# spaceml-org/STARCOP

Hardware: AMD Instinct MI355X
Metric: 512x512 hyperspectral tiles/sec (train fwd+bwd) (higher is better)
Workload: dtype f32; 1 GPU; configs[1]: HyperSTARCOP U-Net (smp.Unet mobilenet_v2, 4ch mag1c+RGB) train step fwd+loss+bwd+Adam, 512x512 tiles, fp32 HIP kernels (3x3 convs: fp32 operands split exactly into 16-bit terms on the matrix cores, fp32 accumulation; see config.precision and DESIGN.md section 2); batch_per_gpu=16, global_batch=16, parallelism=dp1, hipgraph=False, precision=fp32

## Files before the change

### include/starcop_hip.h

```cpp
#ifndef STARCOP_HIP_H
#define STARCOP_HIP_H

#include <stddef.h>
#include <stdint.h>

#ifdef __cplusplus
extern "C" {
#endif

typedef void* sc_stream;

enum sc_status {
  SC_OK = 0,
  SC_ERR_ARG = -1,
  SC_ERR_LAUNCH = -2,
  SC_ERR_NOTPD = -3,
  SC_ERR_NODEV = -4
};

enum sc_src_mode {
  SC_SRC_RAW = 0,
  SC_SRC_AFFINE = 1,
  SC_SRC_BNBWD = 2,
  SC_SRC_NORM = 3
// ... 86 lines not shown
  const float* part; float* dw;
  int32_t nparts, taps, Cout, Cin, CoP, CiP;
  uint64_t total;
} sc_wgrad_pending;
int sc_conv2d_wgrad_mfma_deferred(const sc_wgrad_args* a, sc_wgrad_pending* pending_host, sc_stream stream);
int sc_wgrad_reduce_batch(const sc_wgrad_pending* descs_dev, const uint32_t* block_starts_dev, int n, uint32_t total_blocks,
                          sc_stream stream);
#define SC_PACK_THIN16 5
#define SC_PACK_PW3 6
size_t sc_packed_weight_floats_thin16(int Cout, int Cin, int transpose_flip);
int sc_pack_weights_thin16(const float* w_oihw, float* wpk, int Cout, int Cin, int transpose_flip, sc_stream stream);
int sc_conv3x3_thin16(const sc_conv_args* a, sc_stream stream);

#define SC_PACK_SP 7
size_t sc_packed_weight_floats_sp(int Cout, int Cup, int Cskip);
int sc_pack_weights_sp(const float* w_oihw, float* wpk, int Cout, int Cup, int Cskip, int terms, sc_stream stream);
int sc_sp_stat_rows(int N, int H, int W, int Cout);
int sc_conv3x3_sp(const sc_conv_args* a, sc_stream stream);
#define SC_PACK_SPD 8
size_t sc_packed_weight_floats_spd(int Cout, int Cup, int Cskip_tiles );
int sc_spd_vskip_ok(int Cup, int Cskip);
int sc_pack_weights_spd(const float* w_oihw, float* wpk, int Cout, int CinTotal, int Cup, int vskip, int terms, sc_stream stream);
int sc_conv3x3_sp_dgrad(const sc_conv_args* a, sc_stream stream);
size_t sc_sp_wgrad_workspace_bytes(int N, int H, int W, int Cout, int Cup);
int sc_conv3x3_sp_wgrad(const sc_wgrad_args* a, void* ws, size_t ws_bytes, sc_stream stream);
int sc_wgrad_scatter_cols(const float* src, float* dw, int Cout, int Ccols, int CinTotal, int col_off, sc_stream stream);

size_t sc_wgrad_thin16_workspace_floats(int N, int H, int W, int Cout, int Cin);
int sc_conv3x3_wgrad_thin16(const sc_wgrad_args* a, sc_stream stream);

size_t sc_packed_weight_floats_pw3(int Cout, int Cin, int transpose_flip);
int sc_conv1x1_pw3(const sc_conv_args* a, sc_stream stream);
int sc_conv1x1_pw3_variant(int N, int H, int W, int Cout);
size_t sc_wgrad_pw3_workspace_floats(int N, int H, int W, int Cout, int Cin);
int sc_conv1x1_wgrad_pw3(const sc_wgrad_args* a, sc_wgrad_pending* pending_host, sc_stream stream);
int sc_wgrad_pw3_variant(int N, int H, int W, int Cout, int Cin);

typedef struct sc_irb_args {
  sc_src x;
  const float* wpk_expand;
  const float* cst_expand;
  const float* w_dw;
  const float* cst_dw;
  const float* wpk_project;
  const float* cst_project;
  float* out;
  float* z_absmax;
  int32_t N, Cin, hidden, Cout, H, W, stride, residual;
} sc_irb_args;
int sc_irb_supported(int Cin, int hidden, int Cout, int H, int W, int stride);
int sc_irb_variant(int Cin, int hidden, int Cout, int stride);
int sc_irb_eval(const sc_irb_args* a, sc_stream stream);

typedef struct sc_irt_args {
  sc_src x;
  const float* w_expand;
  const float* w_dw;
  const float* cst_expand;
  int32_t N, Cin, hidden, H, W, stride;
} sc_irt_args;
int sc_irt_supported(int Cin, int hidden, int H, int W, int stride);
int sc_irt_rows(int stage, int N, int H, int W, int stride);
int sc_irt_bwd_rows(int N, int hidden, int H, int W);
size_t sc_irt_bwd_workspace_floats(int N, int Cin, int hidden, int H, int W);
int sc_irt_expand_stats(const sc_irt_args* a, float* stats , sc_stream stream);
int sc_irt_fwd(const sc_irt_args* a, float* d_out , float* stats_d , sc_stream stream);
// ... 532 lines not shown
```

### starcop_amd/_lib.py

```python
import ctypes as C
import os
import subprocess

import torch

_HERE = os.path.dirname(os.path.abspath(__file__))
LIB_PATH = os.path.join(_HERE, "libstarcop_hip.so")
CSRC = os.path.join(_HERE, "csrc")

SC_CST = 8
STAT_CONV3, STAT_CONV1, STAT_DW, STAT_STEM, STAT_BNBWD, STAT_CONV1K, STAT_PW3 = 0, 1, 2, 3, 4, 5, 6

SRC_RAW, SRC_AFFINE, SRC_BNBWD, SRC_NORM = 0, 1, 2, 3
ACT_NONE, ACT_RELU, ACT_RELU6 = 0, 1, 2


class StarcopHipError(RuntimeError):
    pass


class sc_src(C.Structure):
    _fields_ = [("x", C.c_void_p), ("aux", C.c_void_p), ("cst", C.c_void_p),
                ("C", C.c_int32), ("mode", C.c_int32), ("act", C.c_int32), ("up", C.c_int32)]

# ... 317 lines not shown
    "sc_scene_gather_planes": (_i, [C.POINTER(sc_scene_planes_args), _vp]),
    "sc_scene_core_counts": (_i, [_vp, C.c_int64, C.c_int64, _i, _i, C.c_uint32, _vp, _vp, _i, _vp, _vp]),
    "sc_head_conv_fwd_mosaic_prob": (_i, [C.POINTER(sc_src), _vp, _vp, _vp, C.c_int64, _vp, C.c_int64, _i, _i, _vp, C.c_int64, C.c_int64,
                                          C.c_uint32, _f, _vp, _vp, _i, _i, _i, _i, _vp]),
    "sc_connected_components": (_i, [_vp, _i, _vp, _vp, _vp, _sz, _i, _i, _i, _vp]),
    "sc_proposed_mask": (_i, [_vp, C.c_int64, _vp, C.c_int64, _f, _i, _vp, _vp, _sz, _i, _i, _i, _vp]),
    "sc_packed_weight_floats_thin16": (_sz, [_i, _i, _i]),
    "sc_pack_weights_thin16": (_i, [_vp, _vp, _i, _i, _i, _vp]),
    "sc_conv3x3_thin16": (_i, [C.POINTER(sc_conv_args), _vp]),
    "sc_packed_weight_floats_sp": (_sz, [_i, _i, _i]),
    "sc_pack_weights_sp": (_i, [_vp, _vp, _i, _i, _i, _i, _vp]),
    "sc_sp_stat_rows": (_i, [_i, _i, _i, _i]),
    "sc_conv3x3_sp": (_i, [C.POINTER(sc_conv_args), _vp]),
    "sc_packed_weight_floats_spd": (_sz, [_i, _i, _i]),
    "sc_pack_weights_spd": (_i, [_vp, _vp, _i, _i, _i, _i, _i, _vp]),
    "sc_spd_vskip_ok": (_i, [_i, _i]),
    "sc_conv3x3_sp_dgrad": (_i, [C.POINTER(sc_conv_args), _vp]),
    "sc_sp_wgrad_workspace_bytes": (_sz, [_i, _i, _i, _i, _i]),
    "sc_conv3x3_sp_wgrad": (_i, [C.POINTER(sc_wgrad_args), _vp, _sz, _vp]),
    "sc_wgrad_scatter_cols": (_i, [_vp, _vp, _i, _i, _i, _i, _vp]),
    "sc_binary_opening": (_i, [_vp, _f, _i, _vp, _vp, _i, _i, _i, _vp]),
    "sc_threshold_confusion": (_i, [_vp, _vp, _vp, _vp, _i, _i, _vp, _vp, _i, _i, _i, _vp]),
    "sc_gather_augment": (_i, [_vp, _i, _i, _i, _i, _vp, _vp, _vp, _vp, _vp, _vp, _i, _i, _i, _i, _vp, _vp]),
    "sc_tile_window_sums": (_i, [_vp, _i, _i, _i, _vp, _vp, _i, _vp, _vp]),
    "sc_dwconv3x3_bwd_fused": (_i, [C.POINTER(sc_src), C.POINTER(sc_src), _vp, _vp, _vp, _vp, _i, _i, _i, _i, _i, _vp]),
    "sc_dw_variant": (_i, [_i, _i, _i, _i, _i, _i, _i]),
    "sc_wgrad_thin16_workspace_floats": (_sz, [_i, _i, _i, _i, _i]),
    "sc_conv3x3_wgrad_thin16": (_i, [C.POINTER(sc_wgrad_args), _vp]),
    "sc_conv2d_wgrad_mfma_deferred": (_i, [C.POINTER(sc_wgrad_args), C.POINTER(sc_wgrad_pending), _vp]),
    "sc_wgrad_reduce_batch": (_i, [_vp, _vp, _i, C.c_uint32, _vp]),
    "sc_packed_weight_floats_pw3": (_sz, [_i, _i, _i]),
    "sc_conv1x1_pw3": (_i, [C.POINTER(sc_conv_args), _vp]),
    "sc_conv1x1_pw3_variant": (_i, [_i, _i, _i, _i]),
    "sc_wgrad_pw3_workspace_floats": (_sz, [_i, _i, _i, _i, _i]),
    "sc_wgrad_pw3_variant": (_i, [_i, _i, _i, _i, _i]),
    "sc_conv1x1_wgrad_pw3": (_i, [C.POINTER(sc_wgrad_args), C.POINTER(sc_wgrad_pending), _vp]),
    "sc_irb_supported": (_i, [_i, _i, _i, _i, _i, _i]),
    "sc_irb_variant": (_i, [_i, _i, _i, _i]),
    "sc_irb_eval": (_i, [C.POINTER(sc_irb_args), _vp]),
    "sc_irt_supported": (_i, [_i, _i, _i, _i, _i]),
    "sc_irt_rows": (_i, [_i, _i, _i, _i, _i]),
    "sc_irt_bwd_rows": (_i, [_i, _i, _i, _i]),
    "sc_irt_bwd_workspace_floats": (_sz, [_i, _i, _i, _i, _i]),
    "sc_irt_expand_stats": (_i, [C.POINTER(sc_irt_args), _vp, _vp]),
    "sc_irt_fwd": (_i, [C.POINTER(sc_irt_args), _vp, _vp, _vp]),
    "sc_irt_bwd": (_i, [C.POINTER(sc_irt_args), C.POINTER(sc_src), _vp, _vp, _vp, _vp]),
    "sc_irt_xmoments": (_i, [C.POINTER(sc_irt_args), _vp, _vp]),
    "sc_irt_bwd_fix": (_i, [C.POINTER(sc_irt_args), _vp, _vp, _vp, _vp, _i, _vp]),
    "sc_irt_wgrad_finalize": (_i, [C.POINTER(sc_irt_args), _vp, _vp, _vp, _vp]),
    "sc_maxpool2x2": (_i, [C.POINTER(sc_src), _vp, _i, _i, _i, _i, _vp]),
    "sc_upsample_bilinear2x": (_i, [C.POINTER(sc_src), _vp, _i, _i, _i, _i, _vp]),
    "sc_maxpool2x2_bwd": (_i, [C.POINTER(sc_src), _vp, _vp, _i, _i, _i, _i, _i, _vp]),
    "sc_upsample_bilinear2x_bwd": (_i, [_vp, _vp, _i, _i, _i, _i, _vp]),
    "sc_pwreg_param_floats": (_sz, [_i, _i, _i, _i]),
    "sc_pwreg_fwd": (_i, [_vp, _vp, _i, _i, _i, _i, _i, _i, _i, _vp, _vp]),
    "sc_reg_loss": (_i, [_vp, _vp, _sz, _i, _vp, _vp, _vp, _vp]),
    "sc_pwreg_sweep_blocks": (_i, [_i, _i, _i]),
    "sc_pwreg_train_sweep": (_i, [_vp, _vp, _vp, _i, _i, _i, _i, _i, _i, _i, _i, _vp, _vp]),
    "sc_pwreg_finalize": (_i, [_vp, _i, _vp, _i, _i, _i, _i, _d, _vp, _vp, _vp]),
    "sc_panel_minmax": (_i, [_vp, C.POINTER(sc_panel), _i, _vp, _vp]),
    "sc_render_panels": (_i, [_vp, C.POINTER(sc_panel), _i, _vp, _vp, _i, _i, _vp]),
    "sc_component_stats_workspace_bytes": (_sz, [_i, _i, _i, _i, _i]),
    "sc_component_stats": (_i, [C.POINTER(sc_cstats_args), _vp, _sz, _vp]),
    "sc_component_outlines_workspace_bytes": (_sz, [_i, _i, C.c_int64]),
    "sc_component_outlines_rounds": (_i, [C.c_int64]),
    "sc_component_outlines": (_i, [C.POINTER(sc_outline_args), _i, _vp]),
# ... 106 lines not shown
```

### starcop_amd/csrc/conv_pw3.hip

```cpp
#include "sc_split.h"

namespace {

struct PwP {
  SrcD s;
  const uintx4* wpk;
  int NP, HW, K, M, nks, npb;
  float* out; const float* add0; int accum; float* stats;
  const float* bnr_y; const float* bnr_cst; float* bnr_rows; int bnr_act;
};

template <int NCB, int PD, bool BNB>
__global__ __launch_bounds__(256) void k_pw3(const PwP p) {
  constexpr int CW = BNB ? 8 : 2;
  extern __shared__ __attribute__((aligned(16))) float s_cst[];
  const int tid = threadIdx.x, lane = tid & 63, wave = tid >> 6;
  const int l31 = lane & 31, lhi = lane >> 5;
  const int HW = p.HW, K = p.K, M = p.M, nks = p.nks;
  for (int c = tid; c < nks * 16; c += 256) {
    if (BNB) {
      float4 c0 = make_float4(0.f, 0.f, 0.f, 0.f); float c4 = 0.f;
      if (c < K) { c0 = *reinterpret_cast<const float4*>(p.s.cst + (size_t)c * SC_CST); c4 = p.s.cst[(size_t)c * SC_CST + 4]; }
      *reinterpret_cast<float4*>(s_cst + c * 8) = c0;
      *reinterpret_cast<float4*>(s_cst + c * 8 + 4) = make_float4(c4, 0.f, 0.f, 0.f);
// ... 43 lines not shown

  for (int ks0 = 0; ks0 < nks; ks0 += PD) {
#pragma unroll
    for (int s = 0; s < PD; ++s) {
      const int ks = ks0 + s;
      const int kc = ks < nks ? ks : nks - 1;
      const bool live = pok && ks < nks;
      float v[8];
      if (BNB) {
        const float4* q = reinterpret_cast<const float4*>(s_cst + (kc * 16 + lhi * 8) * 8);
#pragma unroll
        for (int j = 0; j < 8; ++j) {
          const float4 c0 = q[2 * j]; const float c4 = q[2 * j + 1].x;
          const float t = sc_pro_bnbwd(xr[s][j], yr[BNB ? s : 0][j], c0.x, c0.y, c0.z, c0.w, c4, lo, hi);
          v[j] = live ? t : 0.f;
        }
      } else {
        const float4* q = reinterpret_cast<const float4*>(s_cst + (kc * 16 + lhi * 8) * 2);
#pragma unroll
        for (int jj = 0; jj < 4; ++jj) {
          const float4 c = q[jj];
          const float t0 = sc_pro_affine(xr[s][2 * jj], c.x, c.y, lo, hi), t1 = sc_pro_affine(xr[s][2 * jj + 1], c.z, c.w, lo, hi);
          v[2 * jj] = live ? t0 : 0.f;
          v[2 * jj + 1] = live ? t1 : 0.f;
        }
      }
      uintx4 a[3];
      split8(v, a);
#pragma unroll
      for (int m = 0; m < NCB; ++m) acc[m] = mfma6(a, br[s][m], acc[m]);
      PW3_ISSUE(s, ks + PD)
    }
  }
#undef PW3_ISSUE

  const bool vec4 = (HW & 3) == 0;
  unsigned ooff[4]; bool ook[4];
#pragma unroll
  for (int j = 0; j < 4; ++j) {
    const int g = pb * 32 + 8 * j + 4 * lhi;
    ook[j] = g < p.NP;
    const int gc = ook[j] ? g : 0;
    const int n_ = gc / HW;
    ooff[j] = (unsigned)(n_ * M) * (unsigned)HW + (unsigned)(gc - n_ * HW);
  }
#pragma unroll
  for (int m = 0; m < NCB; ++m) {
    const int co = (cbase + m) * 32 + l31;
    const bool cok = co < M;
    if (p.stats) {
      float s1 = 0.f, s2 = 0.f;
#pragma unroll
      for (int r = 0; r < 16; ++r) { s1 += acc[m][r]; s2 = fmaf(acc[m][r], acc[m][r], s2); }
      s1 += __shfl_xor(s1, 32, 64);
      s2 += __shfl_xor(s2, 32, 64);
      if (lhi == 0 && cok) *reinterpret_cast<float2*>(p.stats + ((size_t)pb * M + co) * 2) = make_float2(s1, s2);
    }
    if (!cok) continue;
    if (BNB && p.bnr_y != nullptr) {
      const float4 cb = *reinterpret_cast<const float4*>(p.bnr_cst + (size_t)co * SC_CST);
      const float blo = sc_act_lo(p.bnr_act), bhi = sc_act_hi(p.bnr_act);
      float yv[16];
#pragma unroll
      for (int r = 0; r < 16; ++r) yv[r] = 0.f;
      if (vec4) {
#pragma unroll
        for (int j = 0; j < 4; ++j) {
// ... 16 lines not shown
        const float gq = (g < p.NP && yh > blo && yh < bhi) ? acc[m][r] : 0.f;
        s1 += gq;
        s2 = fmaf(gq, (yv[r] - cb.z) * cb.w, s2);
      }
      s1 += __shfl_xor(s1, 32, 64);
      s2 += __shfl_xor(s2, 32, 64);
      if (lhi == 0) *reinterpret_cast<float2*>(p.bnr_rows + ((size_t)pb * M + co) * 2) = make_float2(s1, s2);
    }
    if (vec4) {
#pragma unroll
      for (int j = 0; j < 4; ++j) {
        if (!ook[j]) continue;
        const unsigned idx = ooff[j] + (unsigned)co * (unsigned)HW;
        float4 o = make_float4(acc[m][4 * j], acc[m][4 * j + 1], acc[m][4 * j + 2], acc[m][4 * j + 3]);
        if (p.add0) { const float4 t = *reinterpret_cast<const float4*>(p.add0 + idx); o.x += t.x; o.y += t.y; o.z += t.z; o.w += t.w; }
        if (p.accum) { const float4 t = *reinterpret_cast<const float4*>(p.out + idx); o.x += t.x; o.y += t.y; o.z += t.z; o.w += t.w; }
        *reinterpret_cast<float4*>(p.out + idx) = o;
      }
    } else {
#pragma unroll
      for (int r = 0; r < 16; ++r) {
        const int g = pb * 32 + 8 * (r >> 2) + 4 * lhi + (r & 3);
        if (g >= p.NP) continue;
        const int n_ = g / HW;
        const size_t idx = ((size_t)n_ * M + co) * HW + (g - n_ * HW);
        float o = acc[m][r];
        if (p.add0) o += p.add0[idx];
        if (p.accum) o += p.out[idx];
        p.out[idx] = o;
      }
    }
  }
}

struct PwWP {
  SrcD dy, s;
  int NP, HW, Cout, Cin;
  int ksteps;
  int per_wg;
  int CoP, CiP;
  float* part;
};

template <int TM, int TN, int PD>
__global__ __launch_bounds__(256) void k_pw3_wgrad(const PwWP p) {
  extern __shared__ __attribute__((aligned(16))) float s_red[];
  const int tid = threadIdx.x, lane = tid & 63, wave = tid >> 6;
  const int l31 = lane & 31, lhi = lane >> 5;
  const int HW = p.HW;
  const int mb0 = blockIdx.y * TM, nb0 = blockIdx.z * TN;
  float d_sc[TM], d_sh[TM], d_A[TM], d_B[TM], d_D[TM]; bool d_ok[TM]; unsigned d_c[TM];
  float x_sc[TN], x_sh[TN]; bool x_ok[TN]; unsigned x_c[TN];
  const bool dy_bnb = p.dy.mode == SC_SRC_BNBWD;
#pragma unroll
  for (int m = 0; m < TM; ++m) {
    const int co = (mb0 + m) * 32 + l31;
    d_ok[m] = co < p.Cout;
    d_c[m] = d_ok[m] ? co : 0;
    const float4 c0 = *reinterpret_cast<const float4*>(p.dy.cst + (size_t)d_c[m] * SC_CST);
    d_sc[m] = c0.x; d_sh[m] = c0.y; d_A[m] = c0.z; d_B[m] = c0.w; d_D[m] = p.dy.cst[(size_t)d_c[m] * SC_CST + 4];
  }
#pragma unroll
  for (int q = 0; q < TN; ++q) {
    const int ci = (nb0 + q) * 32 + l31;
    x_ok[q] = ci < p.Cin;
    x_c[q] = x_ok[q] ? ci : 0;
// ... 162 lines not shown
  SC_REQUIRE(((uintptr_t)a->wpk & 15) == 0, "sc_conv1x1_pw3: packed filters must be 16-byte aligned");
  const long NP = (long)a->N * a->H * a->W;
  SC_REQUIRE(NP * (long)(a->Cout > a->src[0].C ? a->Cout : a->src[0].C) < (1L << 32), "sc_conv1x1_pw3: tensor too large for 32-bit element offsets");
  PwP p;
  p.s = to_srcd(a->src[0]);
  if (p.s.mode == SC_SRC_RAW) {
    p.s.cst = sc_identity_cst_table(p.s.C);
    SC_REQUIRE(p.s.cst != nullptr, "sc_conv1x1_pw3: identity constants unavailable (C = %d)", p.s.C);
    p.s.act = SC_ACT_NONE;
  }
  p.wpk = reinterpret_cast<const uintx4*>(a->wpk);
  p.NP = (int)NP; p.HW = a->H * a->W; p.K = a->src[0].C; p.M = a->Cout;
  p.nks = (p.K + 15) / 16;
  p.npb = (int)((NP + 31) / 32);
  p.out = a->out0; p.add0 = a->add0; p.accum = a->accum0; p.stats = a->stats;
  p.bnr_y = nullptr; p.bnr_cst = nullptr; p.bnr_rows = nullptr; p.bnr_act = SC_ACT_NONE;
  if (a->bnr) {
    SC_REQUIRE(p.s.mode == SC_SRC_BNBWD && !a->add0 && !a->accum0 && !a->stats, "sc_conv1x1_pw3: sc_bnr_args go with a data-gradient launch that writes the complete gradient");
    SC_REQUIRE(a->bnr->y && a->bnr->cst && a->bnr->rows && !a->bnr->absmax, "sc_conv1x1_pw3: sc_bnr_args need y, cst and rows (no range hint on this path)");
    p.bnr_y = a->bnr->y; p.bnr_cst = a->bnr->cst; p.bnr_rows = a->bnr->rows; p.bnr_act = a->bnr->act;
  }
  const int MB = (p.M + 31) / 32;
  const int ncb = sc_conv1x1_pw3_variant(a->N, a->H, a->W, a->Cout);
  const bool bnb = p.s.mode == SC_SRC_BNBWD;
  dim3 grid((p.npb + 3) / 4, (MB + ncb - 1) / ncb);
  const size_t lds = (size_t)p.nks * 16 * (bnb ? 8 : 2) * sizeof(float);
  hipStream_t st = (hipStream_t)stream;
#define SC_PW(NCB, PD, B) hipLaunchKernelGGL((k_pw3<NCB, PD, B>), grid, dim3(256), lds, st, p)
  if (ncb == 4) { if (bnb) SC_PW(4, 2, true); else SC_PW(4, 2, false); }
  else if (ncb == 2) { if (bnb) SC_PW(2, 4, true); else SC_PW(2, 4, false); }
  else { if (bnb) SC_PW(1, 4, true); else SC_PW(1, 4, false); }
#undef SC_PW
  SC_LAUNCH_OK("sc_conv1x1_pw3");
  return SC_OK;
}

extern "C" size_t sc_wgrad_pw3_workspace_floats(int N, int H, int W, int Cout, int Cin) {
  const PwWPlan pl = plan_pw3_wgrad(N, H, W, Cout, Cin);
  const size_t E = (size_t)pl.CoP * pl.CiP;
  return (size_t)pl.nparts * E + sc_reduce_scratch_floats(pl.nparts, E);
}

extern "C" int sc_wgrad_pw3_variant(int N, int H, int W, int Cout, int Cin) {
  if (N <= 0 || H <= 0 || W <= 0 || Cout <= 0 || Cin <= 0) return -1;
  const PwWPlan pl = plan_pw3_wgrad(N, H, W, Cout, Cin);
  return 10 * pl.tm + pl.tn;
}

extern "C" int sc_conv1x1_wgrad_pw3(const sc_wgrad_args* a, sc_wgrad_pending* pending, sc_stream stream) {
  SC_REQUIRE(a != nullptr, "sc_conv1x1_wgrad_pw3: null args");
  SC_REQUIRE(a->ks == 1 && a->nsrc == 1, "sc_conv1x1_wgrad_pw3: ks must be 1 with a single source");
  SC_REQUIRE(a->src[0].C == a->Cin && a->dy.C == a->Cout, "sc_conv1x1_wgrad_pw3: channel mismatch");
  SC_REQUIRE(a->dy.up == 0 && a->src[0].up == 0, "sc_conv1x1_wgrad_pw3: sources cannot be upsampled");
  SC_REQUIRE(a->src[0].mode == SC_SRC_RAW || a->src[0].mode == SC_SRC_AFFINE, "sc_conv1x1_wgrad_pw3: input must be a RAW or AFFINE source");
  SC_REQUIRE(a->dy.mode != SC_SRC_NORM && (a->dy.mode != SC_SRC_BNBWD || a->dy.aux), "sc_conv1x1_wgrad_pw3: bad dy source");
  SC_REQUIRE((a->H * a->W) % 8 == 0, "sc_conv1x1_wgrad_pw3: H*W must be a multiple of 8 (got %d)", a->H * a->W);
  const PwWPlan pl = plan_pw3_wgrad(a->N, a->H, a->W, a->Cout, a->Cin);
  const size_t need = sc_wgrad_pw3_workspace_floats(a->N, a->H, a->W, a->Cout, a->Cin);
  SC_REQUIRE(a->part_floats >= need, "sc_conv1x1_wgrad_pw3: workspace too small (%zu < %zu floats)", a->part_floats, need);
  PwWP p;
  p.dy = to_srcd(a->dy); p.s = to_srcd(a->src[0]);
  if (p.dy.mode == SC_SRC_RAW) { p.dy.cst = sc_identity_cst_table(p.dy.C); p.dy.act = SC_ACT_NONE; SC_REQUIRE(p.dy.cst, "sc_conv1x1_wgrad_pw3: identity constants unavailable"); }
  if (p.s.mode == SC_SRC_RAW) { p.s.cst = sc_identity_cst_table(p.s.C); p.s.act = SC_ACT_NONE; SC_REQUIRE(p.s.cst, "sc_conv1x1_wgrad_pw3: identity constants unavailable"); }
  p.NP = a->N * a->H * a->W; p.HW = a->H * a->W; p.Cout = a->Cout; p.Cin = a->Cin;
  p.ksteps = pl.ksteps; p.per_wg = pl.per_wg; p.CoP = pl.CoP; p.CiP = pl.CiP; p.part = a->part;
  dim3 grid(pl.nparts, pl.CoP / (32 * pl.tm), pl.CiP / (32 * pl.tn));
// ... 18 lines not shown
```

### starcop_amd/network.py

```python
import collections
import ctypes as C
import math
import os

import torch
import torch.nn as nn

from . import _lib, scene
from ._lib import (ACT_NONE, ACT_RELU, ACT_RELU6, SC_CST, sc_irb_args, sc_irt_args, SRC_AFFINE, SRC_BNBWD, SRC_NORM, SRC_RAW, STAT_BNBWD, sc_wgrad_pending,
                   PACK_PW3, PACK_SP, PACK_SPD, PACK_THIN16, STAT_PW3, STAT_CONV1, STAT_CONV1K, STAT_CONV3, STAT_DW, STAT_STEM, TERMS_F16X2, check, make_src, ptr, sc_bn_tail, sc_bnr_args,
                   sc_conv_args, sc_wgrad_args, stream)

MBV2_SETTINGS = ((1, 16, 1, 1), (6, 24, 2, 2), (6, 32, 3, 2), (6, 64, 4, 2),
                 (6, 96, 3, 1), (6, 160, 3, 2), (6, 320, 1, 1))
DECODER_CHANNELS = (256, 128, 64, 32, 16)
BN_EPS, BN_MOMENTUM = 1e-5, 0.1
HeadMosaic = collections.namedtuple("HeadMosaic", "win win_host classes prob mask valid fill_bits nodata", defaults=(None,) * 4 + (0, 0.0))


def _conv_bn_act(cin, cout, k, stride=1, groups=1, act="relu6"):
    return nn.Sequential(nn.Conv2d(cin, cout, k, stride, (k - 1) // 2, groups=groups, bias=False),
                         nn.BatchNorm2d(cout, eps=BN_EPS, momentum=BN_MOMENTUM),
                         nn.ReLU6() if act == "relu6" else nn.ReLU())

# ... 145 lines not shown
    if _SP == "0" or Ho % 2 or Wo % 2:
        return False
    if _SP == "all":
        return True
    Hl, Wl = Ho // 2, Wo // 2
    tw = 32 if Wl >= 32 else 16
    wgs = N * (-(-Wl // tw)) * (-(-Hl // (256 // tw))) * (-(-Cout // 32))
    return Cout >= 32 and wgs >= 128


def _use_spd(N, Ho, Wo, Cup, Csk=0):
    if _SP == "0" or Ho % 2 or Wo % 2:
        return False
    return _SP == "all" or Cup >= 128 or (Csk and _lib.load().sc_spd_vskip_ok(Cup, Csk))


def _use_spd_skip_tiles(Cup, Csk):
    if _SP == "all":
        return True
    return _SP != "0" and _SP_SKIPTILES and Cup >= 1024 and -(-Csk // 32) * 3 <= -(-Cup // 128)


def _use_spw(N, Ho, Wo, Cout, Cup):
    if _SP == "0" or Ho % 2 or Wo % 2:
        return False
    return _SP == "all" or Cup >= 512


def _use_ksplit(N, HW, K, M, ks=1):
    if ks != 1:
        return False
    wgs = N * (-(-HW // 128)) * (-(-M // _pick_cot(M, 1)))
    return wgs <= 512 and (K >= 384 or (K >= 192 and wgs <= 256))


class HyperStarcopUNet(nn.Module):

    def __init__(self, in_channels=4, classes=1):
        super().__init__()
        if not (1 <= classes <= self.MAX_CLASSES):
            raise ValueError(f"HyperStarcopUNet: classes must be in [1, {self.MAX_CLASSES}] (sc_head_conv_fwd_k)")
        if not (1 <= in_channels <= self.MAX_IN_CHANNELS):
            raise ValueError(f"HyperStarcopUNet: in_channels must be in [1, {self.MAX_IN_CHANNELS}] (sc_stem_conv_fwd)")
        self.in_channels, self.classes = in_channels, classes
        self.encoder = _Encoder(in_channels)
        self.decoder = _Decoder()
        self.segmentation_head = nn.Sequential(nn.Conv2d(DECODER_CHANNELS[-1], classes, 3, padding=1))
        self.reset_parameters()
        self._ops, self._tensors = self._build_ops()
        self._plans = {}
        self._pflat = self._gflat = None
        self._pack_version = None
        self.register_load_state_dict_post_hook(HyperStarcopUNet._after_load)

    MAX_IN_CHANNELS, MAX_CLASSES = 16, 8
    MAX_TRAIN_IN_CHANNELS, MAX_TRAIN_CLASSES = 8, 1

    @staticmethod
    def _after_load(module, incompatible_keys):
        module.check_split_range()

    FP16_MAX_WEIGHT, FP16_MAX_ACT = 255.0, 32752.0
    range_check_every = 200

    def _split_feeders(self):
        raw, fin = [], []
# ... 211 lines not shown
    class _Plan:
        pass

    def _get_plan(self, N, H, W, need_grad, want_logits=True, want_classes=None):
        want_classes = (not want_logits) if want_classes is None else want_classes
        key = (N, H, W)
        plan = self._plans.get(key)
        dev = self._pflat.device
        if plan is None:
            plan = HyperStarcopUNet._Plan()
            plan.N, plan.H, plan.W = N, H, W
            plan.buf, plan.grad = {}, {}
            f32 = dict(dtype=torch.float32, device=dev)
            lib = _lib.load()
            plan.cst, plan.cstb, plan.stats_v, plan.bsums_v, plan.srows, plan.brows = {}, {}, {}, {}, {}, {}
            kind_of = {"stem": STAT_STEM, "dw": STAT_DW, "conv3": STAT_CONV3, "pw": STAT_CONV1}
            plan.irt, plan.irt_of_dw, plan.irt_rows = {}, {}, {}
            if self.fuse_irt:
                for i_e, (i_dw, i_pr, stride) in self._ir_blocks.items():
                    cv, tin = self._ops[i_e]["conv"], self._ops[i_e]["ins"][0]
                    if tin.kind != "input" and _use_irt(N, cv.in_channels, cv.out_channels, H >> tin.shift, W >> tin.shift, stride):
                        plan.irt[i_e], plan.irt_of_dw[i_dw] = i_dw, i_e
                        te, td = self._ops[i_e]["out"], self._ops[i_dw]["out"]
                        plan.irt_rows[te.name] = lib.sc_irt_rows(0, N, H >> tin.shift, W >> tin.shift, stride)
                        plan.irt_rows[td.name] = lib.sc_irt_rows(1, N, H >> tin.shift, W >> tin.shift, stride)
            irt_e = {self._ops[i]["out"].name for i in plan.irt}
            for op in self._ops:
                t = op["out"]
                if t.kind != "input" and t.name not in plan.buf and t.name not in irt_e and t.name != "logits":
                    plan.buf[t.name] = torch.empty((N, t.C, H >> t.shift, W >> t.shift), **f32)
                if t.bn is not None:
                    Ho, Wo = H >> t.shift, W >> t.shift
                    kind = kind_of[op["type"]]
                    if op["type"] == "pw" and _use_pw3(0, N, Ho * Wo, op["conv"].in_channels, op["conv"].out_channels):
                        kind = STAT_PW3
                    elif op["type"] == "pw" and _use_ksplit(N, Ho * Wo, op["conv"].in_channels, op["conv"].out_channels):
                        kind = STAT_CONV1K
                    plan.srows[t.name] = max(lib.sc_stat_rows(kind, N, Ho, Wo), plan.irt_rows.get(t.name, 0))
                    plan.brows[t.name] = lib.sc_stat_rows(STAT_BNBWD, N, Ho, Wo)
                    plan.stats_v[t.name] = torch.empty(plan.srows[t.name] * t.C * 2, **f32)
                    plan.cst[t.name] = torch.zeros((t.C, SC_CST), **f32)
                    plan.cstb[t.name] = torch.zeros((t.C, SC_CST), **f32)
            plan.irb = {}
            for i_e, (i_dw, i_pr, stride) in self._ir_blocks.items():
                cv_e, cv_p, tin = self._ops[i_e]["conv"], self._ops[i_pr]["conv"], self._ops[i_e]["ins"][0]
                if tin.kind != "input" and _use_irb(N, cv_e.in_channels, cv_e.out_channels, cv_p.out_channels, H >> tin.shift, W >> tin.shift, stride):
                    i_add = i_pr + 1 if (i_pr + 1 < len(self._ops) and self._ops[i_pr + 1]["type"] == "add"
                                         and self._ops[i_pr + 1]["ins"][1] is self._ops[i_pr]["out"]) else None
                    plan.irb[i_e] = (i_dw, i_pr, i_add)
                    lay = getattr(self, "_irb_layers", None)
                    if lay is None:
                        lay = self._irb_layers = set()
                    if not {i_e, i_pr} <= lay:
                        lay.update((i_e, i_pr))
                        self._pack_version = None
                        self._pack_tables = {}
            need = getattr(self, "_pw_need", None)
            if need is None:
                need = self._pw_need = {}
            for i, op in enumerate(self._ops):
                if op["type"] == "pw":
                    hw = (H >> op["out"].shift) * (W >> op["out"].shift)
                    for tflip in (0, 1):
                        cv = op["conv"]
                        lay = "pw3" if _use_pw3(tflip, N, hw, cv.in_channels, cv.out_channels) else "mfma"
                        if lay not in need.setdefault((i, tflip), set()):
                            need[(i, tflip)].add(lay)
                            self._pack_version = None
                            self._pack_tables = {}
            fins = [t.name for t in self._tensors.values() if t.kind == "fin" and t.name != "logits"]
            plan.bn_scratch = torch.empty(64 * 2 * max(t.C for t in self._tensors.values()), dtype=torch.float64, device=dev)
            plan.fin_slot = {n: i for i, n in enumerate(fins)}
            plan.fin_amax = torch.zeros(len(fins), **f32)
            raw_feed = self._split_feeders()[0]
            plan.act_slot = {n: i for i, n in enumerate(raw_feed)}
            plan.act_amax = torch.zeros(max(len(raw_feed), 1), **f32)
            plan.n_eval = 0
            plan.has_grad = False
            self._plans[key] = plan
        if want_logits and "logits" not in plan.buf:
            plan.buf["logits"] = torch.empty((N, self.classes, H, W), dtype=torch.float32, device=dev)
        if want_classes and getattr(plan, "classes", None) is None:
            plan.classes = torch.empty((N, H, W), dtype=torch.uint8, device=dev)
        if need_grad and not plan.has_grad:
            lib = _lib.load()
            f32 = dict(dtype=torch.float32, device=dev)
            ws, up = 0, 0
            n_dw = 0
            irt_e = {self._ops[i]["out"].name for i in plan.irt}
            plan.irt_esums, plan.irt_work = {}, {}
            for i_e in plan.irt:
                cv, tin, te = self._ops[i_e]["conv"], self._ops[i_e]["ins"][0], self._ops[i_e]["out"]
                Hi, Wi = H >> tin.shift, W >> tin.shift
                plan.irt_esums[te.name] = torch.empty(lib.sc_irt_bwd_rows(N, cv.out_channels, Hi, Wi) * cv.out_channels * 2, dtype=torch.float64, device=dev)
                plan.irt_work[te.name] = torch.empty(lib.sc_irt_bwd_workspace_floats(N, cv.in_channels, cv.out_channels, Hi, Wi), **f32)
            for op in self._ops:
                o = op["out"]
                Ho, Wo = H >> o.shift, W >> o.shift
# ... 344 lines not shown
                    xb_ = self._xbound(plan, o)
                    bt.act_bound = xb_.value if xb_ is not None else None
                    check(lib.sc_dwconv3x3_fwd_bn(C.byref(s), ptr(conv.weight), ptr(plan.buf[o.name]), N, o.C,
                                                  H >> tin.shift, W >> tin.shift, op["stride"], stats, C.byref(bt), st))
                    bn_done = True
                else:
                    check(lib.sc_dwconv3x3_fwd(C.byref(s), ptr(conv.weight), ptr(plan.buf[o.name]), N, o.C,
                                               H >> tin.shift, W >> tin.shift, op["stride"], stats, st))
            elif ty in ("pw", "conv3"):
                if ty == "conv3" and self._late_pack_stream is not None:
                    check(lib.sc_stream_wait_stream(st, self._late_pack_stream))
                    self._late_pack_stream = None
                a = sc_conv_args()
                ins = op["ins"]
                a.nsrc = len(ins)
                a.src[0] = self._src_of(plan, ins[0], up=1 if op.get("up") else 0)
                if len(ins) == 2:
                    a.src[1] = self._src_of(plan, ins[1])
                ent = self._wpk[i]
                a.wpk = ent["f"].data_ptr()
                a.N, a.H, a.W, a.Cout = N, Ho, Wo, o.C
                a.ks, a.co_t = conv.kernel_size[0], ent["cot_f"]
                a.out0 = plan.buf[o.name].data_ptr(); a.out1 = None
                a.csplit, a.accum0, a.accum1 = o.C, 0, 0
                a.add0 = None; a.add1 = None
                a.stats = plan.stats_v[o.name].data_ptr() if stats is not None else None
                a.terms = ent["terms_f"]
                if ty == "conv3":
                    for k_, t_ in enumerate(ins):
                        a.xbound[k_] = self._xbound(plan, t_)
                if ty == "pw" and _use_pw3(0, N, Ho * Wo, conv.in_channels, conv.out_channels):
                    fconv = lib.sc_conv1x1_pw3
                    a.wpk = ent["pf"].data_ptr()
                elif (op.get("up") and ent.get("sp") is not None and ent["terms_f"] in _SP_TERMS and self.split_bf16
                      and _use_sp(N, Ho, Wo, o.C)):
                    fconv = lib.sc_conv3x3_sp
                    a.wpk = ent["sp"].data_ptr()
                    srows = lib.sc_sp_stat_rows(N, Ho, Wo, o.C)
                elif ent["tf"] is not None:
                    fconv = lib.sc_conv3x3_thin16
                    a.wpk = ent["tf"].data_ptr()
                elif ent["bx3_f"]:
                    fconv = lib.sc_conv3x3_bx3
                elif _use_ksplit(N, Ho * Wo, conv.in_channels, conv.out_channels, a.ks):
                    fconv = lib.sc_conv1x1_ksplit
                else:
                    fconv = lib.sc_conv2d_mfma
                check(fconv(C.byref(a), st))
            elif ty == "add":
                sa = self._src_of(plan, op["ins"][0])
                sb = self._src_of(plan, op["ins"][1])
                check(lib.sc_add_srcs_absmax(C.byref(sa), C.byref(sb), ptr(plan.buf[o.name]), N, o.C, Ho * Wo,
                                             plan.fin_amax.data_ptr() + 4 * plan.fin_slot[o.name], st))
            elif ty == "head":
                s = self._src_of(plan, op["ins"][0])
                if head == "mosaic":
                    mos = mosaic.classes
                    check(lib.sc_head_conv_fwd_k_mosaic(C.byref(s), ptr(conv.weight), ptr(conv.bias), ptr(mos), mos.shape[0], mos.shape[1],
                                                        mos.stride(0), mosaic.win, mosaic.win_host,
                                                        N, conv.in_channels, self.classes, Ho, Wo, st))
                elif head == "probmosaic":
                    prob, mask, valid = mosaic.prob, mosaic.mask, mosaic.valid
                    ref = prob if prob is not None else mask
                    check(lib.sc_head_conv_fwd_mosaic_prob(
                        C.byref(s), ptr(conv.weight), ptr(conv.bias), ptr(prob), prob.stride(0) if prob is not None else 0,
                        ptr(mask), mask.stride(0) if mask is not None else 0, ref.shape[0], ref.shape[1],
# ... 445 lines not shown
                wfn = lib.sc_conv3x3_wgrad_thin16
            tok = None if wfn is None else self._pb(
                "k_wgrad3_bx3 (+reduce)" if wfn is lib.sc_conv3x3_wgrad_bx3 else
                "k_wgrad_thin_h (+reduce)" if wfn is lib.sc_conv3x3_wgrad_thin16 else f"k_wgrad_mfma<{ks}> (+reduce)", flop)
            if wfn is None:
                pass
            elif ty == "pw" and i in plan.pw_part:
                wa.part = plan.pw_part[i].data_ptr(); wa.part_floats = plan.pw_part[i].numel()
                pend = sc_wgrad_pending()
                wdef = (lib.sc_conv1x1_wgrad_pw3 if _use_pw3(2, N, Ho * Wo, conv.in_channels, conv.out_channels)
                        else lib.sc_conv2d_wgrad_mfma_deferred)
                wgrad_launch(lambda sx, wa=wa, pend=pend, wdef=wdef: check(wdef(C.byref(wa), C.byref(pend), sx)), second=True)
                pw_pending.append(pend)
                if i == last_pw:
                    reduce_pointwise_batch()
            else:
                wgrad_launch(lambda sx, wfn=wfn, wa=wa: check(wfn(C.byref(wa), sx)))
            self._pe(tok)
            if ins[0].kind == "input":
                continue
            ent = self._wpk[i]
            a = sc_conv_args()
            a.nsrc = 1
            a.src[0] = dy
            a.wpk = ent["b"].data_ptr()
            a.N, a.H, a.W, a.Cout = N, Ho, Wo, conv.in_channels
            a.ks, a.co_t = ks, ent["cot_b"]
            a.terms = ent["terms_b"]
            a.absmax = gmax_slot.get(o.name)
            if ent["bx3_b"]:
                conv_dgrad = lib.sc_conv3x3_bx3
            elif ty == "pw" and _use_pw3(1, N, Ho * Wo, conv.in_channels, conv.out_channels):
                conv_dgrad = lib.sc_conv1x1_pw3
                a.wpk = ent["pb"].data_ptr()
            elif _use_ksplit(N, Ho * Wo, conv.out_channels, conv.in_channels, ks):
                conv_dgrad = lib.sc_conv1x1_ksplit
            else:
                conv_dgrad = lib.sc_conv2d_mfma
            a.add0 = None; a.add1 = None; a.stats = None
            a.accum0 = a.accum1 = 0
            bx3_plain = ent["bx3_b"] and not (a.terms == TERMS_F16X2 and (conv.out_channels + 15) // 16 >= 16 and conv.out_channels <= 256)
            gin_elems = N * conv.in_channels * Ho * Wo
            if op.get("up") and ent["bx3_b"]:
                gin_elems -= N * ins[0].C * Ho * Wo * 3 // 4
            thin_b = (ent["tb"] is not None and not op.get("up") and ins[0].name not in written and res_of.get(ins[0].name) is None)
            thin_sd = (ent.get("tsd") is not None and op.get("up") and len(ins) == 1 and a.terms == TERMS_F16X2 and _THIN_SPD and not _BNR
                       and Ho % 2 == 0 and Wo % 2 == 0)
            fle = None
            if (op.get("up") and ent.get("spd") is not None and ent["terms_b"] in _SP_TERMS and self.split_bf16
                    and _use_spd(N, Ho, Wo, ins[0].C, conv.in_channels - ins[0].C)):
                cu_ = ins[0].C
                fle = (2.0 * N * (Ho // 2) * (Wo // 2) * 16 * conv.out_channels * (-(-cu_ // 128) * 128 + (128 * -(-(conv.in_channels - cu_) // 32) if ent["spd_stiles"] else 0))
                       + (0.0 if (ent["spd_vskip"] or ent["spd_stiles"]) else 2.0 * N * Ho * Wo * 9 * conv.out_channels * (conv.in_channels - cu_)))
            tok = self._pb("k_conv3_thin_h (fwd+dgrad)" if (thin_b or thin_sd) else
                           self._bx3_family("dgrad") if ent["bx3_b"] else f"k_conv_mfma<{ks}> (fwd+dgrad)", flop,
                           4.0 * (2 * N * o.C * Ho * Wo + gin_elems + conv.weight.numel()), fle)
            if (op.get("up") and ent.get("spd") is not None and ent["terms_b"] in _SP_TERMS and self.split_bf16
                    and _use_spd(N, Ho, Wo, ins[0].C, conv.in_channels - ins[0].C)):
                if ent["spd_vskip"] or ent["spd_stiles"]:
                    t_up, t_sk = ins
                    a.Cout, a.csplit = conv.in_channels, t_up.C
                    a.wpk = ent["spd"].data_ptr()
                    a.out0, a.out1 = plan.grad[t_up.name].data_ptr(), plan.grad[t_sk.name].data_ptr()
                    a.accum0, a.accum1, a.down0 = (1 if t_up.name in written else 0), (1 if t_sk.name in written else 0), 0
                    check(lib.sc_conv3x3_sp_dgrad(C.byref(a), st))
                    written.add(t_up.name); written.add(t_sk.name)
# ... 191 lines not shown
```

Before: 1439 tiles/s.

## Add intra-block K-split pw3 kernel for deep low-resolution 1x1 convs

```diff
diff --git a/include/starcop_hip.h b/include/starcop_hip.h
--- a/include/starcop_hip.h
+++ b/include/starcop_hip.h
@@ -142,6 +142,8 @@
 size_t sc_packed_weight_floats_pw3(int Cout, int Cin, int transpose_flip);
 int sc_conv1x1_pw3(const sc_conv_args* a, sc_stream stream);
 int sc_conv1x1_pw3_variant(int N, int H, int W, int Cout);
+int sc_conv1x1_pw3_ks(const sc_conv_args* a, sc_stream stream);
+int sc_conv1x1_pw3_ks_variant(int N, int H, int W, int K, int Cout);
 size_t sc_wgrad_pw3_workspace_floats(int N, int H, int W, int Cout, int Cin);
 int sc_conv1x1_wgrad_pw3(const sc_wgrad_args* a, sc_wgrad_pending* pending_host, sc_stream stream);
 int sc_wgrad_pw3_variant(int N, int H, int W, int Cout, int Cin);
diff --git a/starcop_amd/_lib.py b/starcop_amd/_lib.py
--- a/starcop_amd/_lib.py
+++ b/starcop_amd/_lib.py
@@ -373,6 +373,8 @@
     "sc_packed_weight_floats_pw3": (_sz, [_i, _i, _i]),
     "sc_conv1x1_pw3": (_i, [C.POINTER(sc_conv_args), _vp]),
     "sc_conv1x1_pw3_variant": (_i, [_i, _i, _i, _i]),
+    "sc_conv1x1_pw3_ks": (_i, [C.POINTER(sc_conv_args), _vp]),
+    "sc_conv1x1_pw3_ks_variant": (_i, [_i, _i, _i, _i, _i]),
     "sc_wgrad_pw3_workspace_floats": (_sz, [_i, _i, _i, _i, _i]),
     "sc_wgrad_pw3_variant": (_i, [_i, _i, _i, _i, _i]),
     "sc_conv1x1_wgrad_pw3": (_i, [C.POINTER(sc_wgrad_args), C.POINTER(sc_wgrad_pending), _vp]),
diff --git a/starcop_amd/csrc/conv_pw3.hip b/starcop_amd/csrc/conv_pw3.hip
--- a/starcop_amd/csrc/conv_pw3.hip
+++ b/starcop_amd/csrc/conv_pw3.hip
@@ -99,7 +99,6 @@
       PW3_ISSUE(s, ks + PD)
     }
   }
-#undef PW3_ISSUE
 
   const bool vec4 = (HW & 3) == 0;
   unsigned ooff[4]; bool ook[4];
@@ -182,6 +181,138 @@
     }
   }
 }
+
+constexpr int PW3K_PS = 33;
+
+template <int NCB, int PD, bool BNB>
+__global__ __launch_bounds__(256) void k_pw3_ks(const PwP p) {
+  constexpr int CW = BNB ? 8 : 2;
+  extern __shared__ __attribute__((aligned(16))) float s_cst[];
+  const int tid = threadIdx.x, lane = tid & 63, wave = tid >> 6;
+  const int l31 = lane & 31, lhi = lane >> 5;
+  const int HW = p.HW, K = p.K, M = p.M, nks = p.nks;
+  for (int c = tid; c < nks * 16; c += 256) {
+    if (BNB) {
+      float4 c0 = make_float4(0.f, 0.f, 0.f, 0.f); float c4 = 0.f;
+      if (c < K) { c0 = *reinterpret_cast<const float4*>(p.s.cst + (size_t)c * SC_CST); c4 = p.s.cst[(size_t)c * SC_CST + 4]; }
+      *reinterpret_cast<float4*>(s_cst + c * 8) = c0;
+      *reinterpret_cast<float4*>(s_cst + c * 8 + 4) = make_float4(c4, 0.f, 0.f, 0.f);
+    } else {
+      float2 c0 = make_float2(0.f, 0.f);
+      if (c < K) c0 = *reinterpret_cast<const float2*>(p.s.cst + (size_t)c * SC_CST);
+      *reinterpret_cast<float2*>(s_cst + c * 2) = c0;
+    }
+  }
+  __syncthreads();
+  const int pb = blockIdx.x;
+  const int cbase = blockIdx.y * NCB;
+  const float lo = sc_act_lo(p.s.act), hi = sc_act_hi(p.s.act);
+  const int gp = pb * 32 + l31;
+  const bool pok = gp < p.NP;
+  const int gpc = pok ? gp : 0;
+  const int n = gpc / HW, px = gpc - n * HW;
+  const float* xb = p.s.x + ((size_t)n * K) * HW + px;
+  const float* ab = BNB ? p.s.aux + ((size_t)n * K) * HW + px : nullptr;
+  const uintx4* wb = p.wpk + ((size_t)cbase * nks * 3) * 64 + lane;
+
+  float xr[PD][8];
+  float yr[BNB ? PD : 1][8];
+  uintx4 br[PD][NCB][3];
+  floatx16 acc[NCB];
+#pragma unroll
+  for (int m = 0; m < NCB; ++m)
+#pragma unroll
+    for (int r = 0; r < 16; ++r) acc[m][r] = 0.f;
+
+#pragma unroll
+  for (int s = 0; s < PD; ++s) PW3_ISSUE(s, wave + 4 * s)
+
+  for (int ks0 = wave; ks0 < nks; ks0 += 4 * PD) {
+#pragma unroll
+    for (int s = 0; s < PD; ++s) {
+      const int ks = ks0 + 4 * s;
+      const int kc = ks < nks ? ks : nks - 1;
+      const bool live = pok && ks < nks;
+      float v[8];
+      if (BNB) {
+        const float4* q = reinterpret_cast<const float4*>(s_cst + (kc * 16 + lhi * 8) * 8);
+#pragma unroll
+        for (int j = 0; j < 8; ++j) {
+          const float4 c0 = q[2 * j]; const float c4 = q[2 * j + 1].x;
+          const float t = sc_pro_bnbwd(xr[s][j], yr[BNB ? s : 0][j], c0.x, c0.y, c0.z, c0.w, c4, lo, hi);
+          v[j] = live ? t : 0.f;
+        }
+      } else {
+        const float4* q = reinterpret_cast<const float4*>(s_cst + (kc * 16 + lhi * 8) * 2);
+#pragma unroll
+        for (int jj = 0; jj < 4; ++jj) {
+          const float4 c = q[jj];
+          const float t0 = sc_pro_affine(xr[s][2 * jj], c.x, c.y, lo, hi), t1 = sc_pro_affine(xr[s][2 * jj + 1], c.z, c.w, lo, hi);
+          v[2 * jj] = live ? t0 : 0.f;
+          v[2 * jj + 1] = live ? t1 : 0.f;
+        }
+      }
+      uintx4 a[3];
+      split8(v, a);
+#pragma unroll
+      for (int m = 0; m < NCB; ++m) acc[m] = mfma6(a, br[s][m], acc[m]);
+      PW3_ISSUE(s, ks + 4 * PD)
+    }
+  }
+
+  __syncthreads();
+  float* s_red = s_cst;
+#pragma unroll
+  for (int m = 0; m < NCB; ++m)
+#pragma unroll
+    for (int r = 0; r < 16; ++r) s_red[((wave * NCB + m) * 32 + l31) * PW3K_PS + 8 * (r >> 2) + 4 * lhi + (r & 3)] = acc[m][r];
+  __syncthreads();
+  constexpr int WS = NCB * 32 * PW3K_PS;
+  const int cl = wave * 8 + (lane >> 3), g = lane & 7;
+  const int g0 = pb * 32 + 4 * g;
+  const bool vec4 = (HW & 3) == 0;
+#pragma unroll
+  for (int m = 0; m < NCB; ++m) {
+    float o[4];
+#pragma unroll
+    for (int i = 0; i < 4; ++i) {
+      const float* q = s_red + (m * 32 + cl) * PW3K_PS + 4 * g + i;
+      o[i] = ((q[0] + q[WS]) + q[2 * WS]) + q[3 * WS];
+    }
+    const int co = (cbase + m) * 32 + cl;
+    const bool cok = co < M;
+    if (p.stats) {
+      float s1 = (o[0] + o[1]) + (o[2] + o[3]);
+      float s2 = fmaf(o[3], o[3], fmaf(o[2], o[2], fmaf(o[1], o[1], o[0] * o[0])));
+#pragma unroll
+      for (int d = 1; d < 8; d <<= 1) { s1 += __shfl_xor(s1, d, 64); s2 += __shfl_xor(s2, d, 64); }
+      if (g == 0 && cok) *reinterpret_cast<float2*>(p.stats + ((size_t)pb * M + co) * 2) = make_float2(s1, s2);
+    }
+    if (!cok) continue;
+    if (vec4) {
+      if (g0 >= p.NP) continue;
+      const int n_ = g0 / HW;
+      const unsigned idx = (unsigned)(n_ * M + co) * (unsigned)HW + (unsigned)(g0 - n_ * HW);
+      float4 v4 = make_float4(o[0], o[1], o[2], o[3]);
+      if (p.add0) { const float4 t = *reinterpret_cast<const float4*>(p.add0 + idx); v4.x += t.x; v4.y += t.y; v4.z += t.z; v4.w += t.w; }
+      if (p.accum) { const float4 t = *reinterpret_cast<const float4*>(p.out + idx); v4.x += t.x; v4.y += t.y; v4.z += t.z; v4.w += t.w; }
+      *reinterpret_cast<float4*>(p.out + idx) = v4;
+    } else {
+#pragma unroll
+      for (int i = 0; i < 4; ++i) {
+        const int gq = g0 + i;
+        if (gq >= p.NP) continue;
+        const int n_ = gq / HW;
+        const size_t idx = ((size_t)n_ * M + co) * HW + (gq - n_ * HW);
+        float t = o[i];
+        if (p.add0) t += p.add0[idx];
+        if (p.accum) t += p.out[idx];
+        p.out[idx] = t;
+      }
+    }
+  }
+}
+#undef PW3_ISSUE
 
 struct PwWP {
   SrcD dy, s;
@@ -410,6 +541,54 @@
   else { if (bnb) SC_PW(1, 4, true); else SC_PW(1, 4, false); }
 #undef SC_PW
   SC_LAUNCH_OK("sc_conv1x1_pw3");
+  return SC_OK;
+}
+
+extern "C" int sc_conv1x1_pw3_ks_variant(int N, int H, int W, int K, int Cout) {
+  if (N <= 0 || H <= 0 || W <= 0 || K <= 0 || K > 2048 || Cout <= 0) return -1;
+  return Cout > 32 ? 2 : 1;
+}
+
+extern "C" int sc_conv1x1_pw3_ks(const sc_conv_args* a, sc_stream stream) {
+  SC_REQUIRE(a != nullptr, "sc_conv1x1_pw3_ks: null args");
+  SC_REQUIRE(a->ks == 1 && a->nsrc == 1, "sc_conv1x1_pw3_ks: ks must be 1 with a single source");
+  SC_REQUIRE(a->N > 0 && a->H > 0 && a->W > 0 && a->Cout > 0 && a->src[0].C > 0, "sc_conv1x1_pw3_ks: bad shape");
+  SC_REQUIRE(a->csplit == a->Cout && a->out0 && !a->out1 && !a->add1 && !a->accum1 && !a->down0,
+             "sc_conv1x1_pw3_ks: a single plain output (optional add0 / accum0)");
+  SC_REQUIRE(a->src[0].up == 0 && a->src[0].x, "sc_conv1x1_pw3_ks: source cannot be upsampled");
+  SC_REQUIRE(a->src[0].mode != SC_SRC_NORM, "sc_conv1x1_pw3_ks: NORM sources belong to the stem");
+  SC_REQUIRE(a->src[0].mode == SC_SRC_RAW || a->src[0].cst, "sc_conv1x1_pw3_ks: source constants missing");
+  SC_REQUIRE(a->src[0].mode != SC_SRC_BNBWD || a->src[0].aux, "sc_conv1x1_pw3_ks: BNBWD source needs aux");
+  SC_REQUIRE(((uintptr_t)a->wpk & 15) == 0, "sc_conv1x1_pw3_ks: packed filters must be 16-byte aligned");
+  SC_REQUIRE(!a->bnr, "sc_conv1x1_pw3_ks: sc_bnr_args are not taken on the K-split path (sc_conv1x1_pw3 has them)");
+  const long NP = (long)a->N * a->H * a->W;
+  SC_REQUIRE(NP * (long)(a->Cout > a->src[0].C ? a->Cout : a->src[0].C) < (1L << 32), "sc_conv1x1_pw3_ks: tensor too large for 32-bit element offsets");
+  const int ncb = sc_conv1x1_pw3_ks_variant(a->N, a->H, a->W, a->src[0].C, a->Cout);
+  SC_REQUIRE(ncb > 0, "sc_conv1x1_pw3_ks: K = %d is beyond the 2048 channels whose constants fit in LDS", a->src[0].C);
+  PwP p;
+  p.s = to_srcd(a->src[0]);
+  if (p.s.mode == SC_SRC_RAW) {
+    p.s.cst = sc_identity_cst_table(p.s.C);
+    SC_REQUIRE(p.s.cst != nullptr, "sc_conv1x1_pw3_ks: identity constants unavailable (C = %d)", p.s.C);
+    p.s.act = SC_ACT_NONE;
+  }
+  p.wpk = reinterpret_cast<const uintx4*>(a->wpk);
+  p.NP = (int)NP; p.HW = a->H * a->W; p.K = a->src[0].C; p.M = a->Cout;
+  p.nks = (p.K + 15) / 16;
+  p.npb = (int)((NP + 31) / 32);
+  p.out = a->out0; p.add0 = a->add0; p.accum = a->accum0; p.stats = a->stats;
+  p.bnr_y = nullptr; p.bnr_cst = nullptr; p.bnr_rows = nullptr; p.bnr_act = SC_ACT_NONE;
+  const int MB = (p.M + 31) / 32;
+  const bool bnb = p.s.mode == SC_SRC_BNBWD;
+  dim3 grid(p.npb, (MB + ncb - 1) / ncb);
+  const size_t lds_cst = (size_t)p.nks * 16 * (bnb ? 8 : 2) * sizeof(float), lds_red = (size_t)4 * ncb * 32 * PW3K_PS * sizeof(float);
+  const size_t lds = lds_cst > lds_red ? lds_cst : lds_red;
+  hipStream_t st = (hipStream_t)stream;
+#define SC_PWK(NCB, B) hipLaunchKernelGGL((k_pw3_ks<NCB, 4, B>), grid, dim3(256), lds, st, p)
+  if (ncb == 2) { if (bnb) SC_PWK(2, true); else SC_PWK(2, false); }
+  else { if (bnb) SC_PWK(1, true); else SC_PWK(1, false); }
+#undef SC_PWK
+  SC_LAUNCH_OK("sc_conv1x1_pw3_ks");
   return SC_OK;
 }
 
diff --git a/starcop_amd/network.py b/starcop_amd/network.py
--- a/starcop_amd/network.py
+++ b/starcop_amd/network.py
@@ -201,6 +201,21 @@
         return False
     wgs = N * (-(-HW // 128)) * (-(-M // _pick_cot(M, 1)))
     return wgs <= 512 and (K >= 384 or (K >= 192 and wgs <= 256))
+
+
+_PW3_KS = os.environ.get("STARCOP_PW3_KS", "1")
+
+
+def _use_pw3_ks(which, N, HW, K, M):
+    if _PW3_KS == "0" or which not in (0, 1) or K > 2048:
+        return False
+    if _PW3_KS == "all":
+        return True
+    if HW > 1024 or K < 384 or not _use_ksplit(N, HW, K, M):
+        return False
+    MB = -(-M // 32)
+    wgs = -(-N * HW // 32) * (-(-MB // 2))
+    return wgs >= 128 and (MB % 2 == 0 or wgs >= 384)
 
 
 class HyperStarcopUNet(nn.Module):
@@ -478,7 +493,8 @@
                 if t.bn is not None:
                     Ho, Wo = H >> t.shift, W >> t.shift
                     kind = kind_of[op["type"]]
-                    if op["type"] == "pw" and _use_pw3(0, N, Ho * Wo, op["conv"].in_channels, op["conv"].out_channels):
+                    if op["type"] == "pw" and (_use_pw3(0, N, Ho * Wo, op["conv"].in_channels, op["conv"].out_channels)
+                                               or _use_pw3_ks(0, N, Ho * Wo, op["conv"].in_channels, op["conv"].out_channels)):
                         kind = STAT_PW3
                     elif op["type"] == "pw" and _use_ksplit(N, Ho * Wo, op["conv"].in_channels, op["conv"].out_channels):
                         kind = STAT_CONV1K
@@ -509,7 +525,8 @@
                     hw = (H >> op["out"].shift) * (W >> op["out"].shift)
                     for tflip in (0, 1):
                         cv = op["conv"]
-                        lay = "pw3" if _use_pw3(tflip, N, hw, cv.in_channels, cv.out_channels) else "mfma"
+                        k_, m_ = (cv.out_channels, cv.in_channels) if tflip else (cv.in_channels, cv.out_channels)
+                        lay = "pw3" if (_use_pw3(tflip, N, hw, cv.in_channels, cv.out_channels) or _use_pw3_ks(tflip, N, hw, k_, m_)) else "mfma"
                         if lay not in need.setdefault((i, tflip), set()):
                             need[(i, tflip)].add(lay)
                             self._pack_version = None
@@ -920,6 +937,9 @@
                 if ty == "pw" and _use_pw3(0, N, Ho * Wo, conv.in_channels, conv.out_channels):
                     fconv = lib.sc_conv1x1_pw3
                     a.wpk = ent["pf"].data_ptr()
+                elif ty == "pw" and _use_pw3_ks(0, N, Ho * Wo, conv.in_channels, conv.out_channels):
+                    fconv = lib.sc_conv1x1_pw3_ks
+                    a.wpk = ent["pf"].data_ptr()
                 elif (op.get("up") and ent.get("sp") is not None and ent["terms_f"] in _SP_TERMS and self.split_bf16
                       and _use_sp(N, Ho, Wo, o.C)):
                     fconv = lib.sc_conv3x3_sp
@@ -1431,6 +1451,9 @@
                 conv_dgrad = lib.sc_conv3x3_bx3
             elif ty == "pw" and _use_pw3(1, N, Ho * Wo, conv.in_channels, conv.out_channels):
                 conv_dgrad = lib.sc_conv1x1_pw3
+                a.wpk = ent["pb"].data_ptr()
+            elif ty == "pw" and _use_pw3_ks(1, N, Ho * Wo, conv.out_channels, conv.in_channels):
+                conv_dgrad = lib.sc_conv1x1_pw3_ks
                 a.wpk = ent["pb"].data_ptr()
             elif _use_ksplit(N, Ho * Wo, conv.out_channels, conv.in_channels, ks):
                 conv_dgrad = lib.sc_conv1x1_ksplit
```

New measurement: 1457 tiles/s, median of 6. +1.2%, better.
